# VictoriaMetrics/VictoriaLogs

Measured on NVIDIA H100. Metric: log rows scanned/sec (LogsQL phrase+regex), higher is better.
Workload: dtype u8

## Files before the change

victorialogs_b200/csrc/vl_zstd.cu:

```cuda
#include "vl_zstd.h"

#include <algorithm>
#include <array>
#include <atomic>
#include <chrono>
#include <cstdio>
#include <cstdlib>
#include <cstring>
#include <exception>
#include <thread>

#include "vl_engine.h"
#include "vl_zstd.cuh"
#include "vl_zstd_job.h"

namespace vl {

using namespace zs;

struct ZstdDev {
    DevBuf frames, blocks, bstate, huf_tab, fse_tab, huf_state, fse_state, predef, lits, seqs, frame_err, status, lists;
    bool predef_ready = false;
    cudaStream_t xstream = nullptr;
    std::vector<cudaEvent_t> events;
// ... 20 lines not shown
        hpin = nullptr; hpin_cap = 0;
    }
};

static __global__ void k_pull_words(uint4* __restrict__ dst, const uint4* __restrict__ src, size_t n) {
    for (size_t i = (size_t)blockIdx.x * blockDim.x + threadIdx.x; i < n; i += (size_t)gridDim.x * blockDim.x) dst[i] = src[i];
}
void zstd_dev_free(ZstdDev* d) { if (d) { d->release(); delete d; } }

namespace {
inline unsigned cdiv_u(uint64_t a, uint64_t b) { return (unsigned)((a + b - 1) / b); }
}

struct ZstdJob::Impl : ZstdJobImpl {};

ZstdJob::ZstdJob() : m(new Impl) {}
ZstdJob::~ZstdJob() { delete m; }
bool ZstdJob::empty() const { return m->frames.empty(); }
uint64_t ZstdJob::frames() const { return m->frames.size(); }
uint64_t ZstdJob::blocks() const { return m->blocks.size(); }
uint64_t ZstdJob::compressed_blocks() const { return m->n_compressed; }
uint64_t ZstdJob::sequences() const { return m->n_seqs; }
uint64_t ZstdJob::groups() const { return m->groups.size(); }
void ZstdJob::set_dst(uint32_t id, uint64_t arena_off) { m->frames[id].dst = arena_off; }
void ZstdJob::set_group_hook(std::function<void(uint64_t)> f) { m->group_hook = std::move(f); }

void ZstdJob::add_frame(const uint8_t* f, size_t n, uint64_t zoff, uint64_t* regen, uint32_t* id) {
    ZFrame fr{};
    zwalk::parse_frame_into(m->blocks, (uint32_t)m->frames.size(), f, n, zoff, fr);
    *regen = fr.fcs; *id = (uint32_t)m->frames.size();
    m->commit_frame(fr);
}

size_t ZstdJob::add_bytes_block(const uint8_t* p, size_t n, uint64_t zoff, uint64_t* regen, uint32_t* id) {
    ZFrame fr{};
    const size_t used = zwalk::parse_bytes_block_into(m->blocks, (uint32_t)m->frames.size(), p, n, zoff, fr);
    *regen = fr.fcs; *id = (uint32_t)m->frames.size();
    m->commit_frame(fr);
    return used;
}

void ZstdJob::add_values_blocks(const ZValuesBlock* v, size_t n, int threads, ZValuesInfo* info, size_t* bad, std::string* msg) {
    *bad = SIZE_MAX;
    if (!m->frames.empty()) throw BadInput("BUG: add_values_blocks needs an empty job");
    if (threads > 0) { m->walk_values_blocks(v, n, threads, info, bad, msg); return; }
    uint64_t total_seqs = 0;
    if (!group_scale_env()) {
        ZstdJob dry;
        dry.m->limit_scale = 1u << 20;
        for (size_t i = 0; i < n; i++) {
            try {
                uint64_t r = 0; uint32_t id = 0;
                const size_t c1 = dry.add_bytes_block(v[i].p, v[i].n, v[i].zoff, &r, &id);
                dry.add_bytes_block(v[i].p + c1, v[i].n - c1, v[i].zoff + c1, &r, &id);
            } catch (const BadInput&) { break; }
        }
        total_seqs = dry.m->n_seqs;
    }
    auto taper = [&] { if (!group_scale_env()) m->limit_scale = (m->groups.empty() || m->n_seqs > total_seqs - total_seqs / 12) ? 1 : 4; };
    for (size_t i = 0; i < n; i++) {
        try {
            uint32_t f1 = 0, f2 = 0;
            taper();
            const size_t c1 = add_bytes_block(v[i].p, v[i].n, v[i].zoff, &info[i].lens_len, &f1);
            taper();
            const size_t c2 = add_bytes_block(v[i].p + c1, v[i].n - c1, v[i].zoff + c1, &info[i].data_len, &f2);
            if (c1 + c2 != v[i].n) throw BadInput("unexpected non-empty tail after reading bytes block with strings");
        } catch (const BadInput& e) { *bad = i; *msg = e.msg; return; }
    }
    if (!group_scale_env()) m->limit_scale = 1;
}

void ZstdJob::prepare() { m->prepare(); }

void ZstdJob::digest(uint64_t out[4]) const { m->digest(out); }

void ZstdJob::run(vlscan_ctx* ctx, const uint8_t* zsrc, uint8_t* arena) {
    Impl& J = *m;
    if (J.frames.empty()) return;
    auto now = [] { return std::chrono::duration<double>(std::chrono::steady_clock::now().time_since_epoch()).count(); };
    const double t_prep = now();
    J.prepare();
    const double t_lists = now();
    const std::vector<uint32_t>& lists = J.lists;
    if (!ctx->zdev) ctx->zdev = new ZstdDev;
    ZstdDev& D = *ctx->zdev;
    cudaStream_t st = ctx->stream;
    D.frames.ensure(J.frames.size() * sizeof(ZFrame) + 16); D.blocks.ensure(J.blocks.size() * sizeof(ZBlock) + 16); D.bstate.ensure(J.blocks.size() * sizeof(ZBlockState));
    D.frame_err.ensure(J.frames.size() * 4); D.status.ensure(16); D.lists.ensure(lists.size() * 4 + 16);
    D.huf_tab.ensure(std::max<size_t>((size_t)J.max_huf * Z_HUF_TABLE * 2, 16)); D.huf_state.ensure(std::max<size_t>((size_t)J.max_huf * sizeof(ZSlotState), 16));
    D.fse_tab.ensure(std::max<size_t>((size_t)J.max_fse * Z_FSE_SLOT_BYTES, 16)); D.fse_state.ensure(std::max<size_t>((size_t)J.max_fse * sizeof(ZSlotState), 16));
    const size_t lits_stride = (J.max_lits + 64 + 255) / 256 * 256, seqs_stride = std::max<size_t>(J.max_seqs, 1);
    D.lits.ensure(2 * lits_stride); D.seqs.ensure(2 * seqs_stride * 16);
    if (!D.xstream) VL_CUDA(cudaStreamCreateWithFlags(&D.xstream, cudaStreamNonBlocking));
    if (!D.predef_ready) {
        D.predef.ensure(Z_FSE_SLOT_BYTES);
        k_zstd_predef<<<1, 32, 0, st>>>(D.predef.as<uint8_t>());
        VL_CUDA(cudaFuncSetAttribute(k_seq_decode, cudaFuncAttributeMaxDynamicSharedMemorySize, (int)(Z_SEQ_CTA_LANES * (Z_FSE_SLOT_BYTES + Z_LINEBUF))));
        VL_CUDA(cudaFuncSetAttribute(k_huf_decode, cudaFuncAttributeMaxDynamicSharedMemorySize, (int)(Z_HUF_CTA_BLOCKS * Z_HUF_TABLE * 2)));
        ctx->launches++; VL_CUDA(cudaGetLastError());
        D.predef_ready = true;
    }
    {
        auto up16 = [](size_t n) { return (n + 15) / 16 * 16; };
        const size_t nf = up16(J.frames.size() * sizeof(ZFrame)), nb = up16(J.blocks.size() * sizeof(ZBlock)), nl = up16(lists.size() * 4);
        uint8_t* h = (uint8_t*)D.ensure_hpin(nf + nb + nl + 64);
        const double t_cp = now();
        J.spread_copy(h, J.frames.data(), J.frames.size() * sizeof(ZFrame));
        J.spread_copy(h + nf, J.blocks.data(), J.blocks.size() * sizeof(ZBlock));
        if (!lists.empty()) J.spread_copy(h + nf + nb, lists.data(), lists.size() * 4);
        if (getenv("VLSCAN_DEBUG_TIMING")) fprintf(stderr, "[vlscan zstd] host: work lists of %zu launch groups %.1f ms, %.1f MB of tables to pinned memory %.1f ms (%d threads)\n",
                                                   J.groups.size(), 1e3 * (t_lists - t_prep), (nf + nb + nl) / 1e6, 1e3 * (now() - t_cp), std::max(J.threads, 1));
        k_pull_words<<<296, 256, 0, st>>>(D.frames.as<uint4>(), (const uint4*)h, nf / 16); ctx->launches++;
        k_pull_words<<<296, 256, 0, st>>>(D.blocks.as<uint4>(), (const uint4*)(h + nf), nb / 16); ctx->launches++;
        if (nl) { k_pull_words<<<296, 256, 0, st>>>(D.lists.as<uint4>(), (const uint4*)(h + nf + nb), nl / 16); ctx->launches++; }
        VL_CUDA(cudaGetLastError());
    }
    VL_CUDA(cudaMemsetAsync(D.frame_err.p, 0, J.frames.size() * 4, st));
    VL_CUDA(cudaMemsetAsync(D.status.p, 0, 16, st));
    VL_CUDA(cudaMemsetAsync(D.bstate.p, 0, J.blocks.size() * sizeof(ZBlockState), st));
    ZView V{};
    V.src = zsrc; V.arena = arena; V.frames = D.frames.as<ZFrame>(); V.blocks = D.blocks.as<ZBlock>(); V.bstate = D.bstate.as<ZBlockState>();
    V.huf_tab = D.huf_tab.as<uint16_t>(); V.fse_tab = D.fse_tab.as<uint8_t>(); V.huf_state = D.huf_state.as<ZSlotState>(); V.fse_state = D.fse_state.as<ZSlotState>();
    V.predef = D.predef.as<uint8_t>(); V.lits = D.lits.as<uint8_t>(); V.seqs = D.seqs.as<uint4>(); V.frame_err = D.frame_err.as<unsigned int>();
    V.status = D.status.as<unsigned long long>();
    const uint32_t* L = D.lists.as<uint32_t>();
    const bool dbg = getenv("VLSCAN_DEBUG_TIMING") != nullptr;
    static const char* phase_name[6] = {"huf_build", "huf_decode", "fse_build", "seq_decode", "seq_resolve", "execute"};
    std::vector<std::pair<int, std::pair<cudaEvent_t, cudaEvent_t>>> marks;
    int phase = 0;
    static const bool overlap = [] { const char* e = getenv("VLSCAN_ZSTD_OVERLAP"); return !e || atoi(e) != 0; }();
    cudaStream_t xs = overlap ? D.xstream : st;
    cudaStream_t cur_stream = st;
    auto begin = [&](int p) { phase = p; if (dbg) { cudaEvent_t a, b; cudaEventCreate(&a); cudaEventCreate(&b); cudaEventRecord(a, cur_stream); marks.push_back({p, {a, b}}); } };
    auto launched = [&] { ctx->launches++; VL_CUDA(cudaGetLastError()); if (dbg) cudaEventRecord(marks.back().second.second, cur_stream); };
    VL_CUDA(cudaEventRecord(D.event(0), st)); VL_CUDA(cudaStreamWaitEvent(xs, D.event(0), 0));
    size_t gi = 0;
    for (const Group& g : J.groups) {
        uint32_t nh = g.huf_hi - g.huf_lo, nl = g.lit_hi - g.lit_lo, ns = g.seq_hi - g.seq_lo, nf = g.frame_hi - g.frame_lo;
        if (J.group_hook) {
            uint64_t need = 0;
            for (uint32_t i = J.frames[g.frame_lo].blk_lo; i < J.frames[g.frame_hi - 1].blk_hi; i++) need = std::max<uint64_t>(need, J.blocks[i].src + (J.blocks[i].type == ZB_RLE ? 1 : J.blocks[i].size));
            J.group_hook(need);
        }
        ZView W = V;
        W.lits = V.lits + (gi & 1) * lits_stride; W.seqs = V.seqs + (gi & 1) * seqs_stride;
        cudaEvent_t ev_entropy = D.event(1 + 2 * gi), ev_exec = D.event(2 + 2 * gi);
        cur_stream = st;
        if (gi >= 2) VL_CUDA(cudaStreamWaitEvent(st, D.event(2 + 2 * (gi - 2)), 0));
        if (nh) { begin(0); k_huf_build<<<cdiv_u(nh, 4), 128, 0, st>>>(W, L + g.huf_lo, nh); launched(); }
        if (nl) { begin(1); k_huf_decode<<<cdiv_u(nl, Z_HUF_CTA_BLOCKS), Z_HUF_CTA_BLOCKS * 4, Z_HUF_CTA_BLOCKS * Z_HUF_TABLE * 2, st>>>(W, L + g.lit_lo, nl); launched(); }
        if (ns) {
            begin(2); k_fse_build<<<cdiv_u(ns, 64), 64, 0, st>>>(W, L + g.seq_lo, ns); launched();
            begin(3); k_seq_decode<<<cdiv_u(ns, Z_SEQ_CTA_LANES), 64, Z_SEQ_CTA_LANES * (Z_FSE_SLOT_BYTES + Z_LINEBUF), st>>>(W, L + g.seq_lo, ns); launched();
        }
        VL_CUDA(cudaEventRecord(ev_entropy, st));
        VL_CUDA(cudaStreamWaitEvent(xs, ev_entropy, 0));
        cur_stream = xs;
        begin(4); k_seq_resolve<<<cdiv_u(nf, 64), 64, 0, xs>>>(W, g.frame_lo, nf); launched();
        begin(5); k_execute<<<cdiv_u((uint64_t)nf * 32, Z_EXEC_WARPS * 32), Z_EXEC_WARPS * 32, 0, xs>>>(W, L + g.ord_lo, nf); launched();
        VL_CUDA(cudaEventRecord(ev_exec, xs));
        gi++;
    }
    if (gi) VL_CUDA(cudaStreamWaitEvent(st, D.event(2 + 2 * (gi - 1)), 0));
    cur_stream = st;
    if (dbg) {
        VL_CUDA(cudaStreamSynchronize(xs)); VL_CUDA(cudaStreamSynchronize(st));
        float tot[6] = {0, 0, 0, 0, 0, 0};
        for (auto& mk : marks) { float ms = 0; cudaEventElapsedTime(&ms, mk.second.first, mk.second.second); tot[mk.first] += ms; cudaEventDestroy(mk.second.first); cudaEventDestroy(mk.second.second); }
        fprintf(stderr, "[vlscan zstd] %zu groups:", J.groups.size());
        for (int p = 0; p < 6; p++) fprintf(stderr, " %s %.2f ms", phase_name[p], tot[p]);
        fprintf(stderr, "\n");
    }
    (void)phase;
    J.ran = true;
}

void ZstdJob::check(vlscan_ctx* ctx) {
    if (!m->ran) return;
    unsigned long long stt[2] = {0, 0};
    VL_CUDA(cudaMemcpyAsync(stt, ctx->zdev->status.p, 16, cudaMemcpyDeviceToHost, ctx->stream));
    VL_CUDA(cudaStreamSynchronize(ctx->stream));
    if (!stt[0]) return;
    static const char* what[] = {"", "bad Huffman tree description", "bad Huffman stream", "bad FSE table description", "bad sequences bitstream", "match offset beyond the regenerated data",
                                 "regenerated size differs from the frame content size", "bad literals section"};
    throw BadInput(std::string("cannot decompress block: ") + (stt[0] < 8 ? what[stt[0]] : "corrupted frame") + " (frame " + std::to_string(stt[1] - 1) + " of the batch)");
}

}
```

victorialogs_b200/csrc/vl_zstd.cuh:

```cuda
#pragma once
#include <cuda_runtime.h>
#include <stdint.h>
#include "vl_zstd_types.h"

namespace vl {
namespace zs {

struct ZView {
    const uint8_t* src;
    uint8_t* arena;
    const ZFrame* frames; const ZBlock* blocks; ZBlockState* bstate;
    uint16_t* huf_tab; uint8_t* fse_tab; ZSlotState* huf_state; ZSlotState* fse_state;
    const uint8_t* predef;
    uint8_t* lits; uint4* seqs;
    unsigned int* frame_err;
    unsigned long long* status;
};

static __device__ __forceinline__ void zfail(const ZView& V, uint32_t frame, unsigned code) {
    atomicCAS(&V.frame_err[frame], 0u, code);
    atomicMax(&V.status[0], (unsigned long long)code);
    atomicMax(&V.status[1], (unsigned long long)frame + 1);
}

static __device__ __forceinline__ uint64_t ldu64(const uint8_t* p) {
    uintptr_t a = (uintptr_t)p & ~(uintptr_t)7; uint32_t sh = (uint32_t)((uintptr_t)p & 7) * 8;
    uint64_t lo = *(const uint64_t*)a;
    if (!sh) return lo;
    uint64_t hi = *(const uint64_t*)(a + 8);
    return (lo >> sh) | (hi << (64 - sh));
}
static __device__ __forceinline__ uint64_t peek64(const uint8_t* base, int64_t pos) {
    if (pos >= 64) { int junk = (int)((-pos) & 7); return ldu64(base + ((pos + 7) >> 3) - 8) << junk; }
    if (pos <= 0) return 0;
    uint64_t v = 0; int nb = (int)((pos + 7) >> 3);
    for (int i = 0; i < nb; i++) v |= (uint64_t)base[i] << (8 * i);
    return v << (64 - pos);
}
struct BackReader {
    const uint8_t* base; int64_t pos; uint64_t w; int avail;
    __device__ __forceinline__ bool init(const uint8_t* p, uint32_t len) {
        base = p; w = 0; avail = 0; pos = 0;
        if (!len) return false;
        uint32_t last = p[len - 1];
        if (!last) return false;
        pos = (int64_t)len * 8 - (int64_t)(__clz(last) - 23);
        return true;
    }
    __device__ __forceinline__ uint32_t read(int n) {
        if (n == 0) return 0;
        if (n > avail) { w = peek64(base, pos); avail = 57; }
        uint32_t v = (uint32_t)(w >> (64 - n)); w <<= n; avail -= n; pos -= n;
        return v;
    }
};
struct FwdReader {
    const uint8_t* base; uint32_t len; uint32_t pos;
    __device__ __forceinline__ uint32_t read(int n) { uint32_t v = (uint32_t)(ldu64(base + (pos >> 3)) >> (pos & 7)) & ((1u << n) - 1); pos += n; return v; }
    __device__ __forceinline__ bool overrun() const { return ((pos + 7) >> 3) > len; }
};
static __device__ __forceinline__ int hibit(uint32_t v) { return 31 - __clz(v); }

static __device__ uint32_t fse_read_counts(const uint8_t* p, uint32_t len, int max_al, int max_syms, int16_t* freq, int* nsyms, int* al_out) {
    FwdReader r{p, len, 0};
    if (len < 1) return 0;
    int al = 5 + (int)r.read(4);
    if (al > max_al) return 0;
    int remaining = 1 << al, s = 0;
    while (remaining > 0 && s < max_syms) {
        if (r.overrun()) return 0;
        int bits = hibit((uint32_t)remaining + 1) + 1;
        int val = (int)r.read(bits);
        int lower = (1 << (bits - 1)) - 1;
        int thr = (1 << bits) - 1 - (remaining + 1);
        if ((val & lower) < thr) { r.pos -= 1; val &= lower; }
        else if (val > lower) val -= thr;
        int proba = val - 1;
        remaining -= proba < 0 ? -proba : proba;
        freq[s++] = (int16_t)proba;
        if (proba == 0) {
            int rep = (int)r.read(2);
            for (;;) {
                for (int i = 0; i < rep && s < max_syms; i++) freq[s++] = 0;
                if (rep != 3) break;
                if (r.overrun()) return 0;
                rep = (int)r.read(2);
            }
        }
    }
    if (remaining != 0 || r.overrun()) return 0;
    *nsyms = s; *al_out = al;
    return (r.pos + 7) >> 3;
}

static __device__ bool fse_build_table(uint32_t* tab, int al, const int16_t* freq, int nsyms, uint16_t* next) {
    const int size = 1 << al, mask = size - 1;
    int high = size;
    for (int s = 0; s < nsyms; s++) if (freq[s] == -1) { tab[--high] = (uint32_t)s; next[s] = 1; }
    const int step = (size >> 1) + (size >> 3) + 3;
    int pos = 0;
    for (int s = 0; s < nsyms; s++) {
        if (freq[s] <= 0) continue;
        next[s] = (uint16_t)freq[s];
        for (int i = 0; i < freq[s]; i++) { tab[pos] = (uint32_t)s; do { pos = (pos + step) & mask; } while (pos >= high); }
    }
    if (pos != 0) return false;
    for (int i = 0; i < size; i++) {
        uint32_t s = tab[i]; uint32_t nx = next[s]++;
        int nb = al - hibit(nx);
        uint32_t base = (nx << nb) - (uint32_t)size;
        tab[i] = s | ((uint32_t)nb << 8) | (base << 16);
    }
    return true;
}

static __device__ bool fse_build_seq_table(uint16_t* trans, uint8_t* sym, int al, const int16_t* freq, int nsyms, uint16_t* next) {
    const int size = 1 << al, mask = size - 1;
    int high = size;
    for (int s = 0; s < nsyms; s++) if (freq[s] == -1) { sym[--high] = (uint8_t)s; next[s] = 1; }
    const int step = (size >> 1) + (size >> 3) + 3;
    int pos = 0;
    for (int s = 0; s < nsyms; s++) {
        if (freq[s] <= 0) continue;
        next[s] = (uint16_t)freq[s];
        for (int i = 0; i < freq[s]; i++) { sym[pos] = (uint8_t)s; do { pos = (pos + step) & mask; } while (pos >= high); }
    }
    if (pos != 0) return false;
    for (int i = 0; i < size; i++) {
        uint32_t nx = next[sym[i]]++;
        int nb = al - hibit(nx);
        trans[i] = (uint16_t)(((nx << nb) - (uint32_t)size) | ((uint32_t)nb << 12));
    }
    return true;
}

static __device__ const int16_t Z_LL_DEFAULT[36] = {4, 3, 2, 2, 2, 2, 2, 2, 2, 2, 2, 2, 2, 1, 1, 1, 2, 2, 2, 2, 2, 2, 2, 2, 2, 3, 2, 1, 1, 1, 1, 1, -1, -1, -1, -1};
static __device__ const int16_t Z_ML_DEFAULT[53] = {1, 4, 3, 2, 2, 2, 2, 2, 2, 1, 1, 1, 1, 1, 1, 1, 1, 1, 1, 1, 1, 1, 1, 1, 1, 1, 1, 1, 1, 1, 1, 1, 1, 1, 1, 1, 1, 1, 1, 1, 1, 1, 1, 1, 1, 1, -1, -1, -1, -1, -1, -1, -1};
static __device__ const int16_t Z_OF_DEFAULT[29] = {1, 1, 1, 1, 1, 1, 2, 2, 2, 1, 1, 1, 1, 1, 1, 1, 1, 1, 1, 1, 1, 1, 1, 1, -1, -1, -1, -1, -1};
static __device__ const uint32_t Z_LL_BASE[36] = {0, 1, 2, 3, 4, 5, 6, 7, 8, 9, 10, 11, 12, 13, 14, 15, 16, 18, 20, 22, 24, 28, 32, 40, 48, 64, 128, 256, 512, 1024, 2048, 4096, 8192, 16384, 32768, 65536};
static __device__ const uint8_t Z_LL_BITS[36] = {0, 0, 0, 0, 0, 0, 0, 0, 0, 0, 0, 0, 0, 0, 0, 0, 1, 1, 1, 1, 2, 2, 3, 3, 4, 6, 7, 8, 9, 10, 11, 12, 13, 14, 15, 16};
static __device__ const uint32_t Z_ML_BASE[53] = {3, 4, 5, 6, 7, 8, 9, 10, 11, 12, 13, 14, 15, 16, 17, 18, 19, 20, 21, 22, 23, 24, 25, 26, 27, 28, 29, 30, 31, 32, 33, 34, 35, 37, 39, 41, 43, 47, 51, 59, 67, 83, 99, 131, 259, 515, 1027, 2051, 4099, 8195, 16387, 32771, 65539};
static __device__ const uint8_t Z_ML_BITS[53] = {0, 0, 0, 0, 0, 0, 0, 0, 0, 0, 0, 0, 0, 0, 0, 0, 0, 0, 0, 0, 0, 0, 0, 0, 0, 0, 0, 0, 0, 0, 0, 0, 1, 1, 1, 1, 2, 2, 3, 3, 4, 4, 5, 7, 8, 9, 10, 11, 12, 13, 14, 15, 16};

static __global__ void k_zstd_predef(uint8_t* predef) {
    if (threadIdx.x || blockIdx.x) return;
    int16_t f[53]; uint16_t nx[53];
    uint16_t* tr = (uint16_t*)predef; uint8_t* sy = predef + 2 * Z_FSE_ENTRIES;
    for (int i = 0; i < 36; i++) f[i] = Z_LL_DEFAULT[i];
    fse_build_seq_table(tr + Z_FSE_LL, sy + Z_FSE_LL, 6, f, 36, nx);
    for (int i = 0; i < 53; i++) f[i] = Z_ML_DEFAULT[i];
    fse_build_seq_table(tr + Z_FSE_ML, sy + Z_FSE_ML, 6, f, 53, nx);
    for (int i = 0; i < 29; i++) f[i] = Z_OF_DEFAULT[i];
    fse_build_seq_table(tr + Z_FSE_OF, sy + Z_FSE_OF, 5, f, 29, nx);
}

static __global__ void __launch_bounds__(128) k_huf_build(ZView V, const uint32_t* __restrict__ list, uint32_t n) {
    __shared__ uint8_t s_w[4][256];
    __shared__ uint16_t s_start[4][256];
    __shared__ int s_meta[4][4];
    const uint32_t wi = threadIdx.x >> 5, lane = threadIdx.x & 31;
    const uint32_t item = blockIdx.x * 4 + wi;
    if (item >= n) return;
    const uint32_t bi = list[item];
    const ZBlock& B = V.blocks[bi];
    const uint8_t* p = V.src + B.src + B.lit_hdr;
    const uint32_t avail = B.lit_comp;
    uint8_t* w = s_w[wi];
    if (lane == 0) {
        int ok = 1, nw = 0; uint32_t desc = 0;
        if (avail < 1) ok = 0;
        else {
            uint32_t hb = p[0];
            if (hb >= 128) {
                nw = (int)hb - 127; desc = 1 + (uint32_t)(nw + 1) / 2;
                if (desc > avail) ok = 0;
                else for (int i = 0; i < nw; i++) { uint8_t b = p[1 + i / 2]; w[i] = (i & 1) ? (b & 15) : (b >> 4); }
            } else {
                desc = 1 + hb;
                int16_t freq[256]; uint16_t nx[256]; __align__(4) uint32_t tab[64];
                int ns = 0, al = 0;
                uint32_t used = (hb == 0 || desc > avail) ? 0 : fse_read_counts(p + 1, hb, 6, 256, freq, &ns, &al);
                if (!used || used >= hb || !fse_build_table(tab, al, freq, ns, nx)) ok = 0;
                else {
                    BackReader r;
                    if (!r.init(p + 1 + used, hb - used)) ok = 0;
                    else {
                        uint32_t s1 = r.read(al), s2 = r.read(al);
                        for (;;) {
                            if (nw >= 254) { ok = 0; break; }
                            uint32_t e1 = tab[s1]; w[nw++] = (uint8_t)e1; s1 = (e1 >> 16) + r.read((e1 >> 8) & 0xFF);
                            if (r.pos < 0) { w[nw++] = (uint8_t)tab[s2]; break; }
                            if (nw >= 254) { ok = 0; break; }
                            uint32_t e2 = tab[s2]; w[nw++] = (uint8_t)e2; s2 = (e2 >> 16) + r.read((e2 >> 8) & 0xFF);
                            if (r.pos < 0) { w[nw++] = (uint8_t)tab[s1]; break; }
                        }
                    }
                }
            }
        }
        int maxbits = 0;
        if (ok) {
            uint32_t sum = 0;
            for (int i = 0; i < nw; i++) { if (w[i] > 11) { ok = 0; break; } if (w[i]) sum += 1u << (w[i] - 1); }
            if (ok && sum == 0) ok = 0;
            if (ok) {
                maxbits = hibit(sum) + 1;
                uint32_t left = (1u << maxbits) - sum;
                if (maxbits > 11 || (left & (left - 1)) != 0) ok = 0;
                else { w[nw++] = (uint8_t)(hibit(left) + 1); }
            }
        }
        if (ok) {
            uint32_t cnt[13]; for (int i = 0; i < 13; i++) cnt[i] = 0;
            for (int i = 0; i < nw; i++) cnt[w[i]]++;
            uint32_t nxt[13]; uint32_t acc = 0;
            for (int k = 1; k <= maxbits; k++) { nxt[k] = acc; acc += cnt[k] << (k - 1); }
            for (int i = 0; i < nw; i++) if (w[i]) { s_start[wi][i] = (uint16_t)nxt[w[i]]; nxt[w[i]] += 1u << (w[i] - 1); }
        }
        s_meta[wi][0] = nw; s_meta[wi][1] = maxbits; s_meta[wi][2] = ok;
        V.bstate[bi].huf_desc_len = desc;
    }
    __syncwarp();
    if (!s_meta[wi][2]) { if (lane == 0) zfail(V, B.frame, ZERR_HUF_DESC); return; }
    const int nw = s_meta[wi][0], maxbits = s_meta[wi][1];
    uint16_t* tab = V.huf_tab + (size_t)B.huf_own * Z_HUF_TABLE;
    for (int s = (int)lane; s < nw; s += 32) {
        uint32_t ww = w[s];
        if (!ww) continue;
        uint32_t len = 1u << (ww - 1), st = s_start[wi][s];
        uint16_t e = (uint16_t)(s | ((maxbits + 1 - ww) << 8));
        for (uint32_t k = 0; k < len; k++) tab[st + k] = e;
    }
    if (lane == 0) V.huf_state[B.huf_own].huf_maxbits = (uint8_t)maxbits;
}

static const uint32_t Z_HUF_CTA_BLOCKS = 56;
static __global__ void __launch_bounds__(Z_HUF_CTA_BLOCKS * 4) k_huf_decode(ZView V, const uint32_t* __restrict__ list, uint32_t n) {
    extern __shared__ uint16_t s_tab[];
    const uint32_t local = threadIdx.x >> 2, k = threadIdx.x & 3;
    const uint32_t first = blockIdx.x * Z_HUF_CTA_BLOCKS;
    const uint32_t here = min(Z_HUF_CTA_BLOCKS, n - first);
    for (uint32_t it = 0; it < here; it++) {
        const ZBlock& Bt = V.blocks[list[first + it]];
        const uint32_t entries = 1u << V.huf_state[Bt.huf_slot].huf_maxbits;
        const uint4* g = (const uint4*)(V.huf_tab + (size_t)Bt.huf_slot * Z_HUF_TABLE);
        uint4* d = (uint4*)(s_tab + (size_t)it * Z_HUF_TABLE);
        for (uint32_t e = threadIdx.x; e < entries / 8; e += blockDim.x) d[e] = g[e];
        if (entries < 8 && threadIdx.x == 0) d[0] = g[0];
    }
    __syncthreads();
    if (local >= here) return;
    const uint32_t bi = list[first + local];
    const ZBlock& B = V.blocks[bi];
    if (V.frame_err[B.frame]) return;
    if (B.lit_streams == 1 && k) return;
    const uint32_t maxbits = V.huf_state[B.huf_slot].huf_maxbits;
    const uint16_t* tab = s_tab + (size_t)local * Z_HUF_TABLE;
    const uint32_t desc = B.lit_type == ZL_COMPRESSED ? V.bstate[bi].huf_desc_len : 0;
    if (maxbits == 0 || desc > B.lit_comp) { zfail(V, B.frame, ZERR_HUF_STREAM); return; }
    const uint8_t* s = V.src + B.src + B.lit_hdr + desc;
    uint32_t total = B.lit_comp - desc, len, nout;
    uint8_t* out = V.lits + B.lit_off;
    if (B.lit_streams == 1) { len = total; nout = B.lit_regen; }
    else {
        if (total < 6) { if (!k) zfail(V, B.frame, ZERR_HUF_STREAM); return; }
        uint32_t s1 = s[0] | (s[1] << 8), s2 = s[2] | (s[3] << 8), s3 = s[4] | (s[5] << 8);
        if ((uint64_t)6 + s1 + s2 + s3 > total) { if (!k) zfail(V, B.frame, ZERR_HUF_STREAM); return; }
        uint32_t seg = (B.lit_regen + 3) / 4;
        if (3 * seg > B.lit_regen) { if (!k) zfail(V, B.frame, ZERR_HUF_STREAM); return; }
        uint32_t off = 6 + (k > 0 ? s1 : 0) + (k > 1 ? s2 : 0) + (k > 2 ? s3 : 0);
        len = k == 0 ? s1 : k == 1 ? s2 : k == 2 ? s3 : total - 6 - s1 - s2 - s3;
        s += off; out += (size_t)k * seg; nout = k < 3 ? seg : B.lit_regen - 3 * seg;
    }
    if (!len || !s[len - 1]) { zfail(V, B.frame, ZERR_HUF_STREAM); return; }
    int64_t pos = (int64_t)len * 8 - (int64_t)(__clz((uint32_t)s[len - 1]) - 23);
    const int sh = 64 - (int)maxbits;
    uint32_t i = 0;
    while (i < nout && (((uintptr_t)(out + i)) & 7) && pos >= 0) { const uint32_t e = tab[peek64(s, pos) >> sh]; pos -= (int64_t)(e >> 8); out[i++] = (uint8_t)e; }
    if (nout - i >= 8 && pos >= 128) {
        const uint64_t* org = (const uint64_t*)((uintptr_t)s & ~(uintptr_t)7);
        const uint32_t s0 = (uint32_t)((uintptr_t)s & 7) * 8;
        uint32_t ab = s0 + (uint32_t)pos;
        uint32_t k = (ab - 1) >> 6;
        uint64_t hi = org[k], lo = org[(int32_t)k - 1], n1 = org[(int32_t)k - 2], n2 = org[(int32_t)k - 3];
        const uint32_t sh32 = 32 - maxbits;
        while (nout - i >= 8 && ab - s0 >= 128) {
            uint64_t acc = 0;
#pragma unroll
            for (int half = 0; half < 2; half++) {
                const uint32_t sft = (0u - ab) & 63u;
                const bool up = sft < 32;
                const uint32_t a = up ? (uint32_t)(hi >> 32) : (uint32_t)hi, b = up ? (uint32_t)hi : (uint32_t)(lo >> 32), c = up ? (uint32_t)(lo >> 32) : (uint32_t)lo;
                uint32_t ch = __funnelshift_l(b, a, sft), cl = __funnelshift_l(c, b, sft);
                uint32_t used = 0;
#pragma unroll
                for (int q = 0; q < 4; q++) {
                    const uint32_t e = tab[ch >> sh32];
                    const uint32_t nb = e >> 8;
                    ch = __funnelshift_l(cl, ch, nb); cl <<= nb;
                    used += nb;
                    acc |= (uint64_t)(e & 0xFF) << (8 * (4 * half + q));
                }
                ab -= used;
                const uint32_t k2 = (ab - 1) >> 6;
                if (k2 != k) { hi = lo; lo = n1; n1 = n2; n2 = org[(int32_t)k2 - 3]; k = k2; }
            }
            *(uint64_t*)(out + i) = acc; i += 8;
        }
        pos = (int64_t)ab - (int64_t)s0;
    }
    while (i < nout && pos >= 0) { const uint32_t e = tab[peek64(s, pos) >> sh]; pos -= (int64_t)(e >> 8); out[i++] = (uint8_t)e; }
    if (i != nout || pos != 0) zfail(V, B.frame, ZERR_HUF_STREAM);
}

static __global__ void __launch_bounds__(64) k_fse_build(ZView V, const uint32_t* __restrict__ list, uint32_t n) {
    const uint32_t t = blockIdx.x * blockDim.x + threadIdx.x;
    if (t >= n) return;
    const uint32_t bi = list[t];
    const ZBlock& B = V.blocks[bi];
    const uint8_t* p = V.src + B.src;
    uint32_t off = B.seq_hdr + 1;
    bool ok = off <= B.size && (B.modes & 3) == 0;
    int16_t freq[53]; uint16_t nx[53];
    ZSlotState st{0, 0, 0, 0};
    for (int k = 0; k < 3 && ok; k++) {
        int mode = k == 0 ? (B.modes >> 6) & 3 : k == 1 ? (B.modes >> 4) & 3 : (B.modes >> 2) & 3;
        int max_al = k == 1 ? 8 : 9, max_syms = k == 0 ? 36 : k == 1 ? 32 : 53;
        uint32_t toff = k == 0 ? Z_FSE_LL : k == 1 ? Z_FSE_OF : Z_FSE_ML;
        int al = 0;
        if (mode == 1) {
            if (off + 1 > B.size) { ok = false; break; }
            uint32_t sym = p[off++];
            if ((int)sym >= max_syms) { ok = false; break; }
            uint8_t* slot = V.fse_tab + (size_t)B.fse_own * Z_FSE_SLOT_BYTES;
            ((uint16_t*)slot)[toff] = 0; slot[2 * Z_FSE_ENTRIES + toff] = (uint8_t)sym;
        } else if (mode == 2) {
            int ns = 0;
            uint32_t used = off < B.size ? fse_read_counts(p + off, B.size - off, max_al, max_syms, freq, &ns, &al) : 0;
            uint8_t* slot = V.fse_tab + (size_t)B.fse_own * Z_FSE_SLOT_BYTES;
            if (!used || !fse_build_seq_table((uint16_t*)slot + toff, slot + 2 * Z_FSE_ENTRIES + toff, al, freq, ns, nx)) { ok = false; break; }
            off += used;
        } else continue;
        if (k == 0) st.ll_al = (uint8_t)al; else if (k == 1) st.of_al = (uint8_t)al; else st.ml_al = (uint8_t)al;
    }
    if (!ok || off > B.size) { zfail(V, B.frame, ZERR_FSE_DESC); return; }
    if (B.fse_own != Z_PREDEF) V.fse_state[B.fse_own] = st;
    V.bstate[bi].seq_bits_off = off;
}

static const uint32_t Z_SEQ_CTA_LANES = 56;
static const uint32_t Z_LINEBUF = 272;
static const uint32_t Z_SEQ_LEAD = 160;
static __device__ __forceinline__ uint32_t lds_u32(uint32_t sa) { uint32_t v; asm volatile("ld.shared.u32 %0, [%1];" : "=r"(v) : "r"(sa)); return v; }
static __device__ __forceinline__ uint32_t bfe_u32(uint32_t a, uint32_t pos, uint32_t len) { uint32_t d; asm("bfe.u32 %0, %1, %2, %3;" : "=r"(d) : "r"(a), "r"(pos), "r"(len)); return d; }
static __device__ __forceinline__ uint32_t top_bits(uint32_t x, uint32_t n) { return __funnelshift_rc(x, 0u, 32u - n); }
struct SeqLane {
    const uint8_t* gorg;
    uint32_t ring;
    uint32_t p;
    uint32_t fc;
    const uint16_t* tr; const uint8_t* sy; const uint32_t* llv; const uint32_t* mlv;
    uint32_t sl, so, sm, r1, r2, r3, ndirty, sum_ll, sum_ml, sticky;
    uint4* out;
    __device__ __forceinline__ void fetch_chunk() {
        fc--;
        const uint32_t sa = ring + ((fc & 15u) << 4);
        const uint8_t* g = gorg + (size_t)fc * 16;
        asm volatile("cp.async.cg.shared.global [%0], [%1], 16;" ::"r"(sa), "l"(g) : "memory");
    }
    __device__ __forceinline__ void window(uint32_t& c2, uint32_t& c1, uint32_t& c0) const {
        const uint32_t k = (p - 1u) >> 5, s = (0u - p) & 31u;
        const uint32_t w3 = lds_u32(ring + ((k << 2) & 252u)), w2 = lds_u32(ring + (((k - 1u) << 2) & 252u));
        const uint32_t w1 = lds_u32(ring + (((k - 2u) << 2) & 252u)), w0 = lds_u32(ring + (((k - 3u) << 2) & 252u));
        c2 = __funnelshift_l(w2, w3, s); c1 = __funnelshift_l(w1, w2, s); c0 = __funnelshift_l(w0, w1, s);
    }
    template <bool LAST>
    __device__ __forceinline__ void step() {
        const uint32_t tl = tr[sl], to = tr[so], tm = tr[sm];
        const uint32_t oc = sy[so], vl = llv[sy[sl]], vm = mlv[sy[sm]];
        if (p < fc * 128u + Z_SEQ_LEAD * 8u && fc > 0) fetch_chunk();
        asm volatile("cp.async.commit_group;\n\tcp.async.wait_group 3;" ::: "memory");
        uint32_t c2, c1, c0;
        window(c2, c1, c0);
        const uint32_t nL = vl >> 24, nM = vm >> 24, n2 = nM + nL;
        const uint32_t ov = (1u << oc) + top_bits(c2, oc);
        const uint32_t v2 = top_bits(__funnelshift_l(c1, c2, oc), n2);
        const uint32_t ml = (vm & 0xFFFFFFu) + (v2 >> nL), ll = (vl & 0xFFFFFFu) + bfe_u32(v2, 0, nL);
        const uint32_t o3 = oc + n2;
        if (!LAST) {
            const uint32_t bL = tl >> 12, bM = tm >> 12, bO = to >> 12, n3 = bL + bM + bO;
            const bool up = o3 < 32;
            const uint32_t v3 = top_bits(__funnelshift_l(up ? c1 : c0, up ? c2 : c1, o3), n3);
            sl = Z_FSE_LL + (tl & 0xFFFu) + (v3 >> (bM + bO));
            sm = Z_FSE_ML + (tm & 0xFFFu) + bfe_u32(v3, bO, bM);
            so = Z_FSE_OF + (to & 0xFFFu) + bfe_u32(v3, 0, bO);
            p -= o3 + n3;
        } else p -= o3;
        uint32_t o;
        if (ov > 3) { o = ov - 3; r3 = r2; r2 = r1; r1 = o; }
        else {
            const uint32_t idx = ov + (ll == 0 ? 1 : 0);
            if (idx == 1) o = r1;
            else {
                o = idx == 2 ? r2 : idx == 3 ? r3 : (r1 == 0xFFFFFFFFu ? r1 : r1 - 1);
                if (idx != 2) r3 = r2;
                r2 = r1; r1 = o;
            }
        }
        ndirty += (r1 | r2 | r3) >> 31;
        *out++ = make_uint4(ll, ml, o, ov);
        sum_ll += ll; sum_ml += ml;
        sticky |= p | sum_ll | sum_ml;
    }
};
static __global__ void __launch_bounds__(64) k_seq_decode(ZView V, const uint32_t* __restrict__ list, uint32_t n) {
    extern __shared__ __align__(16) uint8_t s_fse[];
    __shared__ uint32_t s_llv[36], s_mlv[53];
    const uint32_t first = blockIdx.x * Z_SEQ_CTA_LANES;
    const uint32_t here = min(Z_SEQ_CTA_LANES, n - first);
    if (threadIdx.x < 36) s_llv[threadIdx.x] = Z_LL_BASE[threadIdx.x] | ((uint32_t)Z_LL_BITS[threadIdx.x] << 24);
    if (threadIdx.x < 53) s_mlv[threadIdx.x] = Z_ML_BASE[threadIdx.x] | ((uint32_t)Z_ML_BITS[threadIdx.x] << 24);
    for (uint32_t it = 0; it < here; it++) {
        const ZBlock& Bt = V.blocks[list[first + it]];
        const uint4* src_ll = (const uint4*)(Bt.ll_slot == Z_PREDEF ? V.predef : V.fse_tab + (size_t)Bt.ll_slot * Z_FSE_SLOT_BYTES);
        const uint4* src_ml = (const uint4*)(Bt.ml_slot == Z_PREDEF ? V.predef : V.fse_tab + (size_t)Bt.ml_slot * Z_FSE_SLOT_BYTES);
        const uint4* src_of = (const uint4*)(Bt.of_slot == Z_PREDEF ? V.predef : V.fse_tab + (size_t)Bt.of_slot * Z_FSE_SLOT_BYTES);
        uint4* d = (uint4*)(s_fse + (size_t)it * Z_FSE_SLOT_BYTES);
        for (uint32_t c = threadIdx.x; c < Z_FSE_SLOT_BYTES / 16; c += blockDim.x) {
            const uint4* src = c < 64 ? src_ll : c < 128 ? src_ml : c < 160 ? src_of : c < 192 ? src_ll : c < 224 ? src_ml : src_of;
            d[c] = src[c];
        }
    }
    __syncthreads();
    if (threadIdx.x >= here) return;
    const uint32_t bi = list[first + threadIdx.x];
    const ZBlock& B = V.blocks[bi];
    if (V.frame_err[B.frame]) return;
    const uint32_t off = V.bstate[bi].seq_bits_off;
    const int ll_al = B.ll_slot == Z_PREDEF ? 6 : V.fse_state[B.ll_slot].ll_al;
    const int of_al = B.of_slot == Z_PREDEF ? 5 : V.fse_state[B.of_slot].of_al;
    const int ml_al = B.ml_slot == Z_PREDEF ? 6 : V.fse_state[B.ml_slot].ml_al;
    if (off >= B.size) { zfail(V, B.frame, ZERR_SEQ_STREAM); return; }
    const uint64_t st = B.src + off;
    const uint32_t len = B.size - off;
    const uint32_t last = V.src[st + len - 1];
    if (!last) { zfail(V, B.frame, ZERR_SEQ_STREAM); return; }
    SeqLane L;
    const uint64_t org = (st & ~255ull) - 256;
    const uint32_t s0 = (uint32_t)(st - org) * 8;
    L.gorg = V.src + org;
    L.ring = (uint32_t)__cvta_generic_to_shared(s_fse + (size_t)Z_SEQ_CTA_LANES * Z_FSE_SLOT_BYTES + (size_t)threadIdx.x * Z_LINEBUF);
    L.p = s0 + len * 8 - (uint32_t)(__clz(last) - 23);
    L.fc = ((L.p - 1u) >> 7) + 1u;
#pragma unroll
    for (int q = 0; q < 12; q++) L.fetch_chunk();
    asm volatile("cp.async.commit_group;\n\tcp.async.wait_group 0;" ::: "memory");
    L.tr = (const uint16_t*)(s_fse + (size_t)threadIdx.x * Z_FSE_SLOT_BYTES);
    L.sy = s_fse + (size_t)threadIdx.x * Z_FSE_SLOT_BYTES + 2 * Z_FSE_ENTRIES;
    L.llv = s_llv; L.mlv = s_mlv;
    {
        uint32_t c2, c1, c0;
        L.window(c2, c1, c0);
        L.sl = Z_FSE_LL + top_bits(c2, ll_al);
        L.so = Z_FSE_OF + top_bits(__funnelshift_l(c1, c2, ll_al), of_al);
        L.sm = Z_FSE_ML + top_bits(__funnelshift_l(c1, c2, ll_al + of_al), ml_al);
        L.p -= ll_al + of_al + ml_al;
        (void)c0;
    }
    const uint32_t DIRTY = 0xFFFFFFFFu;
    L.r1 = B.rep_known ? 1 : DIRTY; L.r2 = B.rep_known ? 4 : DIRTY; L.r3 = B.rep_known ? 8 : DIRTY;
    L.ndirty = 0; L.sum_ll = 0; L.sum_ml = 0; L.sticky = L.p;
    L.out = V.seqs + B.seq_base;
    const uint32_t nseq = B.nseq;
    for (uint32_t i = 0; i + 1 < nseq; i++) L.step<false>();
    if (nseq) L.step<true>();
    asm volatile("cp.async.wait_group 0;" ::: "memory");
    if ((L.sticky >> 31) || L.p != s0 || L.sum_ll > B.lit_regen) { zfail(V, B.frame, ZERR_SEQ_STREAM); return; }
    ZBlockState& S = V.bstate[bi];
    S.out_len = B.lit_regen + L.sum_ml;
    S.clean_from = B.rep_known ? 0 : L.ndirty + 1;
    S.rep[0] = L.r1; S.rep[1] = L.r2; S.rep[2] = L.r3;
}

static __global__ void __launch_bounds__(64) k_seq_resolve(ZView V, uint32_t frame_lo, uint32_t nframes) {
    const uint32_t t = blockIdx.x * blockDim.x + threadIdx.x;
    if (t >= nframes) return;
    const uint32_t f = frame_lo + t;
    if (V.frame_err[f]) return;
    const ZFrame& F = V.frames[f];
    uint64_t out = 0;
    uint32_t r1 = 1, r2 = 4, r3 = 8;
    for (uint32_t bi = F.blk_lo; bi < F.blk_hi; bi++) {
        const ZBlock& B = V.blocks[bi];
        ZBlockState& S = V.bstate[bi];
        S.out_base = (uint32_t)out;
        if (B.type != ZB_COMPRESSED) { out += B.size; S.out_len = B.size; continue; }
        if (!B.nseq) { S.out_len = B.lit_regen; out += B.lit_regen; }
        else {
            uint4* __restrict__ sq = V.seqs + B.seq_base;
            const uint32_t redo = min(S.clean_from, B.nseq);
            for (uint32_t i = 0; i < redo; i++) {
                uint4 q = sq[i];
                uint32_t ll = q.x, ov = q.w, o;
                if (ov > 3) { o = ov - 3; r3 = r2; r2 = r1; r1 = o; }
                else {
                    uint32_t idx = ov + (ll == 0 ? 1 : 0);
                    if (idx == 1) o = r1;
                    else {
                        o = idx == 2 ? r2 : idx == 3 ? r3 : r1 - 1;
                        if (idx != 2) r3 = r2;
                        r2 = r1; r1 = o;
                    }
                }
                sq[i].z = o;
            }
            if (S.clean_from <= B.nseq) { r1 = S.rep[0]; r2 = S.rep[1]; r3 = S.rep[2]; }
            out += S.out_len;
        }
        if (out > F.fcs) { zfail(V, f, ZERR_SIZE); return; }
    }
    if (out != F.fcs) zfail(V, f, ZERR_SIZE);
}

static const uint32_t Z_RING = 4096;
static const uint32_t Z_EXEC_WARPS = 4;
static __device__ __forceinline__ uint32_t ldu32(const uint8_t* p) {
    const uintptr_t a = (uintptr_t)p & ~(uintptr_t)3;
    const uint32_t lo = *(const uint32_t*)a, hi = *(const uint32_t*)(a + 4);
    return __funnelshift_r(lo, hi, (uint32_t)((uintptr_t)p & 3) * 8);
}
static __global__ void __launch_bounds__(128) k_execute(ZView V, const uint32_t* __restrict__ order, uint32_t nframes) {
    __shared__ __align__(16) uint8_t s_ring[Z_EXEC_WARPS][Z_RING];
    const uint32_t wid = (blockIdx.x * blockDim.x + threadIdx.x) >> 5, lane = threadIdx.x & 31;
    if (wid >= nframes) return;
    const uint32_t f = order[wid];
    if (V.frame_err[f]) return;
    const ZFrame& F = V.frames[f];
    uint8_t* dst = V.arena + F.dst;
    uint8_t* ring = s_ring[threadIdx.x >> 5];
    const uint32_t abase = (uint32_t)(uintptr_t)dst;
#define VL_RIDX(p) ((abase + (p)) & (Z_RING - 1))
#define VL_RING(p) ring[VL_RIDX(p)]
    uint32_t ring_lo = 0;
    for (uint32_t bi = F.blk_lo; bi < F.blk_hi; bi++) {
        const ZBlock& B = V.blocks[bi];
        const uint32_t blk_base = V.bstate[bi].out_base;
        const uint8_t* p = V.src + B.src;
        if (B.type == ZB_RAW) { for (uint32_t k = lane; k < B.size; k += 32) { uint8_t v = p[k]; dst[blk_base + k] = v; VL_RING(blk_base + k) = v; } __syncwarp(); continue; }
        if (B.type == ZB_RLE) { uint8_t v = p[0]; for (uint32_t k = lane; k < B.size; k += 32) { dst[blk_base + k] = v; VL_RING(blk_base + k) = v; } __syncwarp(); continue; }
        const uint8_t* lit = B.lit_type == ZL_RAW ? p + B.lit_hdr : V.lits + B.lit_off;
        const bool lit_rle = B.lit_type == ZL_RLE;
        const uint8_t rle_byte = lit_rle ? p[B.lit_hdr] : 0;
        const uint4* __restrict__ sq = V.seqs + B.seq_base;
        uint32_t lit_run = 0, out_run = blk_base;
        uint4 qn = lane < B.nseq ? sq[lane] : make_uint4(0, 0, 0, 0);
        for (uint32_t g = 0; g < B.nseq; g += 32) {
            const uint4 q = qn;
            qn = g + 32 + lane < B.nseq ? sq[g + 32 + lane] : make_uint4(0, 0, 0, 0);
            uint32_t il = q.x, io = q.x + q.y;
#pragma unroll
            for (int d = 1; d < 32; d <<= 1) { uint32_t a = __shfl_up_sync(0xffffffffu, il, d), b = __shfl_up_sync(0xffffffffu, io, d); if ((int)lane >= d) { il += a; io += b; } }
            const uint32_t lit_start = il - q.x;
            const uint32_t o_start = io - q.x - q.y;
            const uint32_t T = __shfl_sync(0xffffffffu, il, 31), O = __shfl_sync(0xffffffffu, io, 31);
            const uint32_t gend = out_run + O;
            const uint32_t cnt = min(32u, B.nseq - g);
            const uint32_t ml = q.y, off = q.z, amd = out_run + o_start + q.x;
            if (__any_sync(0xffffffffu, lane < cnt && (off == 0 || off > amd))) { if (lane == 0) zfail(V, f, ZERR_OFFSET); return; }
            const uint32_t s_src = amd - off, e_src = s_src + min(ml, off);
            int dep = -1;
            {
                uint32_t lo = 0;
#pragma unroll
                for (int s = 16; s; s >>= 1) { uint32_t v = __shfl_sync(0xffffffffu, amd, (lo + s - 1) & 31); if ((lo + s - 1) < cnt && v < e_src) lo += s; }
                const uint32_t ci = (lo - 1) & 31;
                const uint32_t ca = __shfl_sync(0xffffffffu, amd, ci), cm = __shfl_sync(0xffffffffu, ml, ci);
                if (lo > 0 && ca + cm > s_src) dep = (int)lo - 1;
            }
            if (O < Z_RING) {
                uint32_t cl = (q.x + 3) >> 2, cm = (ml + 3) >> 2;
#pragma unroll
                for (int d = 1; d < 32; d <<= 1) { uint32_t a = __shfl_up_sync(0xffffffffu, cl, d), b = __shfl_up_sync(0xffffffffu, cm, d); if ((int)lane >= d) { cl += a; cm += b; } }
                const uint32_t CL = __shfl_sync(0xffffffffu, cl, 31);
                const uint32_t pk = lit_start | (o_start << 16);
                const uint8_t* lsrc = lit + lit_run;
                for (uint32_t c0 = 0; c0 < CL; c0 += 128) {
                    uint32_t w[4], at[4], nb[4];
#pragma unroll
                    for (int u = 0; u < 4; u++) {
                        nb[u] = 0; w[u] = 0; at[u] = 0;
                        if (c0 + 32 * u >= CL) continue;
                        const uint32_t c = c0 + 32 * u + lane;
                        uint32_t lo = 0;
#pragma unroll
                        for (int s = 16; s; s >>= 1) { uint32_t x = __shfl_sync(0xffffffffu, cl, (lo + s - 1) & 31); if (x <= c) lo += s; }
                        const uint32_t jc = __shfl_sync(0xffffffffu, cl, lo & 31), jl = __shfl_sync(0xffffffffu, q.x, lo & 31), jp = __shfl_sync(0xffffffffu, pk, lo & 31);
                        if (c < CL) {
                            const uint32_t b0 = (c - (jc - ((jl + 3) >> 2))) * 4;
                            nb[u] = min(4u, jl - b0);
                            w[u] = lit_rle ? rle_byte * 0x01010101u : ldu32(lsrc + (jp & 0xFFFF) + b0);
                            at[u] = out_run + (jp >> 16) + b0;
                        }
                    }
#pragma unroll
                    for (int u = 0; u < 4; u++) {
#pragma unroll
                        for (int t = 0; t < 4; t++) if ((uint32_t)t < nb[u]) VL_RING(at[u] + t) = (uint8_t)(w[u] >> (8 * t));
                    }
                }
                __syncwarp();
                uint32_t cur = 0;
                while (cur < cnt) {
// ... 103 lines not shown
```

victorialogs_b200/csrc/vl_zstd_types.h:

```cpp
#pragma once
#include <stdint.h>

namespace vl {
namespace zs {

enum { ZERR_NONE = 0, ZERR_HUF_DESC = 1, ZERR_HUF_STREAM = 2, ZERR_FSE_DESC = 3, ZERR_SEQ_STREAM = 4, ZERR_OFFSET = 5, ZERR_SIZE = 6, ZERR_LITERALS = 7 };
enum { ZB_RAW = 0, ZB_RLE = 1, ZB_COMPRESSED = 2 };
enum { ZL_RAW = 0, ZL_RLE = 1, ZL_COMPRESSED = 2, ZL_TREELESS = 3 };
static const uint32_t Z_PREDEF = 0xFFFFFFFFu;
static const uint32_t Z_HUF_TABLE = 2048;
static const uint32_t Z_FSE_LL = 0, Z_FSE_ML = 512, Z_FSE_OF = 1024, Z_FSE_ENTRIES = 1280, Z_FSE_SLOT_BYTES = 3 * 1280;

struct ZFrame {
    uint64_t dst;
    uint64_t fcs;
    uint32_t blk_lo, blk_hi;
};
struct ZBlock {
    uint64_t src;
    uint64_t lit_off;
    uint64_t seq_base;
    uint32_t size;
    uint32_t frame;
    uint32_t lit_hdr;
    uint32_t lit_regen, lit_comp;
    uint32_t nseq;
    uint32_t seq_hdr;
    uint32_t huf_slot;
    uint32_t huf_own;
    uint32_t fse_own;
    uint32_t ll_slot, of_slot, ml_slot;
    uint8_t type, lit_type, lit_streams, modes;
    uint8_t rep_known;
    uint8_t pad[3];
};
struct ZBlockState {
    uint32_t huf_desc_len;
    uint32_t seq_bits_off;
    uint32_t out_len;
    uint32_t out_base;
    uint32_t clean_from;
    uint32_t rep[3];
};
struct ZSlotState { uint8_t huf_maxbits, ll_al, of_al, ml_al; };

}
}
```

Measured before the change: 21.70 billion.

## Pack FSE sequence tables into 16-bit entries and stage them with cp.async

The FSE sequence decode table now stores symbol and next-state counter in one 16-bit entry, and the bit count and base are derived at decode time with clz. The separate symbol byte array goes away and per-slot shared memory shrinks from 3840 to 2560 bytes. With the smaller slots the kernel raises lanes per CTA from 56 to 80 and threads from 64 to 96. Table staging is reworked so each block's slot pointers are gathered in parallel and the copies use cp.async instead of a serial per-block loop. The decode step does a few more ALU operations per sequence in exchange for fewer shared loads and a smaller footprint.

After: 21.70 billion, median of 6. Within noise of the previous version (-0.0%).

```diff
diff --git a/victorialogs_b200/csrc/vl_zstd.cu b/victorialogs_b200/csrc/vl_zstd.cu
--- a/victorialogs_b200/csrc/vl_zstd.cu
+++ b/victorialogs_b200/csrc/vl_zstd.cu
@@ -196,7 +196,7 @@
         if (nl) { begin(1); k_huf_decode<<<cdiv_u(nl, Z_HUF_CTA_BLOCKS), Z_HUF_CTA_BLOCKS * 4, Z_HUF_CTA_BLOCKS * Z_HUF_TABLE * 2, st>>>(W, L + g.lit_lo, nl); launched(); }
         if (ns) {
             begin(2); k_fse_build<<<cdiv_u(ns, 64), 64, 0, st>>>(W, L + g.seq_lo, ns); launched();
-            begin(3); k_seq_decode<<<cdiv_u(ns, Z_SEQ_CTA_LANES), 64, Z_SEQ_CTA_LANES * (Z_FSE_SLOT_BYTES + Z_LINEBUF), st>>>(W, L + g.seq_lo, ns); launched();
+            begin(3); k_seq_decode<<<cdiv_u(ns, Z_SEQ_CTA_LANES), Z_SEQ_CTA_THREADS, Z_SEQ_CTA_LANES * (Z_FSE_SLOT_BYTES + Z_LINEBUF), st>>>(W, L + g.seq_lo, ns); launched();
         }
         VL_CUDA(cudaEventRecord(ev_entropy, st));
         VL_CUDA(cudaStreamWaitEvent(xs, ev_entropy, 0));
diff --git a/victorialogs_b200/csrc/vl_zstd.cuh b/victorialogs_b200/csrc/vl_zstd.cuh
--- a/victorialogs_b200/csrc/vl_zstd.cuh
+++ b/victorialogs_b200/csrc/vl_zstd.cuh
@@ -114,22 +114,21 @@
     return true;
 }
 
-static __device__ bool fse_build_seq_table(uint16_t* trans, uint8_t* sym, int al, const int16_t* freq, int nsyms, uint16_t* next) {
+static __device__ bool fse_build_seq_table(uint16_t* tab, int al, const int16_t* freq, int nsyms, uint16_t* next) {
     const int size = 1 << al, mask = size - 1;
     int high = size;
-    for (int s = 0; s < nsyms; s++) if (freq[s] == -1) { sym[--high] = (uint8_t)s; next[s] = 1; }
+    for (int s = 0; s < nsyms; s++) if (freq[s] == -1) { tab[--high] = (uint16_t)s; next[s] = 1; }
     const int step = (size >> 1) + (size >> 3) + 3;
     int pos = 0;
     for (int s = 0; s < nsyms; s++) {
         if (freq[s] <= 0) continue;
         next[s] = (uint16_t)freq[s];
-        for (int i = 0; i < freq[s]; i++) { sym[pos] = (uint8_t)s; do { pos = (pos + step) & mask; } while (pos >= high); }
+        for (int i = 0; i < freq[s]; i++) { tab[pos] = (uint16_t)s; do { pos = (pos + step) & mask; } while (pos >= high); }
     }
     if (pos != 0) return false;
     for (int i = 0; i < size; i++) {
-        uint32_t nx = next[sym[i]]++;
-        int nb = al - hibit(nx);
-        trans[i] = (uint16_t)(((nx << nb) - (uint32_t)size) | ((uint32_t)nb << 12));
+        const uint32_t s = tab[i];
+        tab[i] = (uint16_t)(next[s]++ | (s << 10));
     }
     return true;
 }
@@ -145,13 +144,13 @@
 static __global__ void k_zstd_predef(uint8_t* predef) {
     if (threadIdx.x || blockIdx.x) return;
     int16_t f[53]; uint16_t nx[53];
-    uint16_t* tr = (uint16_t*)predef; uint8_t* sy = predef + 2 * Z_FSE_ENTRIES;
+    uint16_t* tab = (uint16_t*)predef;
     for (int i = 0; i < 36; i++) f[i] = Z_LL_DEFAULT[i];
-    fse_build_seq_table(tr + Z_FSE_LL, sy + Z_FSE_LL, 6, f, 36, nx);
+    fse_build_seq_table(tab + Z_FSE_LL, 6, f, 36, nx);
     for (int i = 0; i < 53; i++) f[i] = Z_ML_DEFAULT[i];
-    fse_build_seq_table(tr + Z_FSE_ML, sy + Z_FSE_ML, 6, f, 53, nx);
+    fse_build_seq_table(tab + Z_FSE_ML, 6, f, 53, nx);
     for (int i = 0; i < 29; i++) f[i] = Z_OF_DEFAULT[i];
-    fse_build_seq_table(tr + Z_FSE_OF, sy + Z_FSE_OF, 5, f, 29, nx);
+    fse_build_seq_table(tab + Z_FSE_OF, 5, f, 29, nx);
 }
 
 static __global__ void __launch_bounds__(128) k_huf_build(ZView V, const uint32_t* __restrict__ list, uint32_t n) {
@@ -332,13 +331,13 @@
             if (off + 1 > B.size) { ok = false; break; }
             uint32_t sym = p[off++];
             if ((int)sym >= max_syms) { ok = false; break; }
-            uint8_t* slot = V.fse_tab + (size_t)B.fse_own * Z_FSE_SLOT_BYTES;
-            ((uint16_t*)slot)[toff] = 0; slot[2 * Z_FSE_ENTRIES + toff] = (uint8_t)sym;
+            uint16_t* slot = (uint16_t*)(V.fse_tab + (size_t)B.fse_own * Z_FSE_SLOT_BYTES);
+            slot[toff] = (uint16_t)(1u | (sym << 10));
         } else if (mode == 2) {
             int ns = 0;
             uint32_t used = off < B.size ? fse_read_counts(p + off, B.size - off, max_al, max_syms, freq, &ns, &al) : 0;
-            uint8_t* slot = V.fse_tab + (size_t)B.fse_own * Z_FSE_SLOT_BYTES;
-            if (!used || !fse_build_seq_table((uint16_t*)slot + toff, slot + 2 * Z_FSE_ENTRIES + toff, al, freq, ns, nx)) { ok = false; break; }
+            uint16_t* slot = (uint16_t*)(V.fse_tab + (size_t)B.fse_own * Z_FSE_SLOT_BYTES);
+            if (!used || !fse_build_seq_table(slot + toff, al, freq, ns, nx)) { ok = false; break; }
             off += used;
         } else continue;
         if (k == 0) st.ll_al = (uint8_t)al; else if (k == 1) st.of_al = (uint8_t)al; else st.ml_al = (uint8_t)al;
@@ -348,7 +347,8 @@
     V.bstate[bi].seq_bits_off = off;
 }
 
-static const uint32_t Z_SEQ_CTA_LANES = 56;
+static const uint32_t Z_SEQ_CTA_LANES = 80;
+static const uint32_t Z_SEQ_CTA_THREADS = 96;
 static const uint32_t Z_LINEBUF = 272;
 static const uint32_t Z_SEQ_LEAD = 160;
 static __device__ __forceinline__ uint32_t lds_u32(uint32_t sa) { uint32_t v; asm volatile("ld.shared.u32 %0, [%1];" : "=r"(v) : "r"(sa)); return v; }
@@ -359,7 +359,8 @@
     uint32_t ring;
     uint32_t p;
     uint32_t fc;
-    const uint16_t* tr; const uint8_t* sy; const uint32_t* llv; const uint32_t* mlv;
+    const uint16_t* tab; const uint32_t* llv; const uint32_t* mlv;
+    uint32_t aL, aM, aO, kL, kM, kO;
     uint32_t sl, so, sm, r1, r2, r3, ndirty, sum_ll, sum_ml, sticky;
     uint4* out;
     __device__ __forceinline__ void fetch_chunk() {
@@ -376,8 +377,8 @@
     }
     template <bool LAST>
     __device__ __forceinline__ void step() {
-        const uint32_t tl = tr[sl], to = tr[so], tm = tr[sm];
-        const uint32_t oc = sy[so], vl = llv[sy[sl]], vm = mlv[sy[sm]];
+        const uint32_t el = tab[sl], eo = tab[so], em = tab[sm];
+        const uint32_t oc = eo >> 10, vl = llv[el >> 10], vm = mlv[em >> 10];
         if (p < fc * 128u + Z_SEQ_LEAD * 8u && fc > 0) fetch_chunk();
         asm volatile("cp.async.commit_group;\n\tcp.async.wait_group 3;" ::: "memory");
         uint32_t c2, c1, c0;
@@ -388,12 +389,13 @@
         const uint32_t ml = (vm & 0xFFFFFFu) + (v2 >> nL), ll = (vl & 0xFFFFFFu) + bfe_u32(v2, 0, nL);
         const uint32_t o3 = oc + n2;
         if (!LAST) {
-            const uint32_t bL = tl >> 12, bM = tm >> 12, bO = to >> 12, n3 = bL + bM + bO;
+            const uint32_t xL = el & 0x3FFu, xM = em & 0x3FFu, xO = eo & 0x3FFu;
+            const uint32_t bL = (uint32_t)__clz(xL) + aL, bM = (uint32_t)__clz(xM) + aM, bO = (uint32_t)__clz(xO) + aO, n3 = bL + bM + bO;
             const bool up = o3 < 32;
             const uint32_t v3 = top_bits(__funnelshift_l(up ? c1 : c0, up ? c2 : c1, o3), n3);
-            sl = Z_FSE_LL + (tl & 0xFFFu) + (v3 >> (bM + bO));
-            sm = Z_FSE_ML + (tm & 0xFFFu) + bfe_u32(v3, bO, bM);
-            so = Z_FSE_OF + (to & 0xFFFu) + bfe_u32(v3, 0, bO);
+            sl = (xL << bL) + kL + (v3 >> (bM + bO));
+            sm = (xM << bM) + kM + bfe_u32(v3, bO, bM);
+            so = (xO << bO) + kO + bfe_u32(v3, 0, bO);
             p -= o3 + n3;
         } else p -= o3;
         uint32_t o;
@@ -413,24 +415,28 @@
         sticky |= p | sum_ll | sum_ml;
     }
 };
-static __global__ void __launch_bounds__(64) k_seq_decode(ZView V, const uint32_t* __restrict__ list, uint32_t n) {
+static __global__ void __launch_bounds__(Z_SEQ_CTA_THREADS) k_seq_decode(ZView V, const uint32_t* __restrict__ list, uint32_t n) {
     extern __shared__ __align__(16) uint8_t s_fse[];
     __shared__ uint32_t s_llv[36], s_mlv[53];
     const uint32_t first = blockIdx.x * Z_SEQ_CTA_LANES;
     const uint32_t here = min(Z_SEQ_CTA_LANES, n - first);
     if (threadIdx.x < 36) s_llv[threadIdx.x] = Z_LL_BASE[threadIdx.x] | ((uint32_t)Z_LL_BITS[threadIdx.x] << 24);
     if (threadIdx.x < 53) s_mlv[threadIdx.x] = Z_ML_BASE[threadIdx.x] | ((uint32_t)Z_ML_BITS[threadIdx.x] << 24);
-    for (uint32_t it = 0; it < here; it++) {
-        const ZBlock& Bt = V.blocks[list[first + it]];
-        const uint4* src_ll = (const uint4*)(Bt.ll_slot == Z_PREDEF ? V.predef : V.fse_tab + (size_t)Bt.ll_slot * Z_FSE_SLOT_BYTES);
-        const uint4* src_ml = (const uint4*)(Bt.ml_slot == Z_PREDEF ? V.predef : V.fse_tab + (size_t)Bt.ml_slot * Z_FSE_SLOT_BYTES);
-        const uint4* src_of = (const uint4*)(Bt.of_slot == Z_PREDEF ? V.predef : V.fse_tab + (size_t)Bt.of_slot * Z_FSE_SLOT_BYTES);
-        uint4* d = (uint4*)(s_fse + (size_t)it * Z_FSE_SLOT_BYTES);
-        for (uint32_t c = threadIdx.x; c < Z_FSE_SLOT_BYTES / 16; c += blockDim.x) {
-            const uint4* src = c < 64 ? src_ll : c < 128 ? src_ml : c < 160 ? src_of : c < 192 ? src_ll : c < 224 ? src_ml : src_of;
-            d[c] = src[c];
-        }
-    }
+    __shared__ const uint8_t* s_slot[3][Z_SEQ_CTA_LANES];
+    if (threadIdx.x < here) {
+        const ZBlock& Bt = V.blocks[list[first + threadIdx.x]];
+        s_slot[0][threadIdx.x] = Bt.ll_slot == Z_PREDEF ? V.predef : V.fse_tab + (size_t)Bt.ll_slot * Z_FSE_SLOT_BYTES;
+        s_slot[1][threadIdx.x] = Bt.ml_slot == Z_PREDEF ? V.predef : V.fse_tab + (size_t)Bt.ml_slot * Z_FSE_SLOT_BYTES;
+        s_slot[2][threadIdx.x] = Bt.of_slot == Z_PREDEF ? V.predef : V.fse_tab + (size_t)Bt.of_slot * Z_FSE_SLOT_BYTES;
+    }
+    __syncthreads();
+    const uint32_t s_base = (uint32_t)__cvta_generic_to_shared(s_fse);
+    for (uint32_t u = threadIdx.x; u < here * (Z_FSE_SLOT_BYTES / 16); u += blockDim.x) {
+        const uint32_t it = u / (Z_FSE_SLOT_BYTES / 16), c = u - it * (Z_FSE_SLOT_BYTES / 16);
+        const uint8_t* g = s_slot[c < 64 ? 0 : c < 128 ? 1 : 2][it] + (size_t)c * 16;
+        asm volatile("cp.async.cg.shared.global [%0], [%1], 16;" ::"r"(s_base + u * 16), "l"(g) : "memory");
+    }
+    asm volatile("cp.async.commit_group;\n\tcp.async.wait_group 0;" ::: "memory");
     __syncthreads();
     if (threadIdx.x >= here) return;
     const uint32_t bi = list[first + threadIdx.x];
@@ -455,9 +461,10 @@
 #pragma unroll
     for (int q = 0; q < 12; q++) L.fetch_chunk();
     asm volatile("cp.async.commit_group;\n\tcp.async.wait_group 0;" ::: "memory");
-    L.tr = (const uint16_t*)(s_fse + (size_t)threadIdx.x * Z_FSE_SLOT_BYTES);
-    L.sy = s_fse + (size_t)threadIdx.x * Z_FSE_SLOT_BYTES + 2 * Z_FSE_ENTRIES;
+    L.tab = (const uint16_t*)(s_fse + (size_t)threadIdx.x * Z_FSE_SLOT_BYTES);
     L.llv = s_llv; L.mlv = s_mlv;
+    L.aL = (uint32_t)(ll_al - 31); L.aM = (uint32_t)(ml_al - 31); L.aO = (uint32_t)(of_al - 31);
+    L.kL = Z_FSE_LL - (1u << ll_al); L.kM = Z_FSE_ML - (1u << ml_al); L.kO = Z_FSE_OF - (1u << of_al);
     {
         uint32_t c2, c1, c0;
         L.window(c2, c1, c0);
diff --git a/victorialogs_b200/csrc/vl_zstd_types.h b/victorialogs_b200/csrc/vl_zstd_types.h
--- a/victorialogs_b200/csrc/vl_zstd_types.h
+++ b/victorialogs_b200/csrc/vl_zstd_types.h
@@ -9,7 +9,7 @@
 enum { ZL_RAW = 0, ZL_RLE = 1, ZL_COMPRESSED = 2, ZL_TREELESS = 3 };
 static const uint32_t Z_PREDEF = 0xFFFFFFFFu;
 static const uint32_t Z_HUF_TABLE = 2048;
-static const uint32_t Z_FSE_LL = 0, Z_FSE_ML = 512, Z_FSE_OF = 1024, Z_FSE_ENTRIES = 1280, Z_FSE_SLOT_BYTES = 3 * 1280;
+static const uint32_t Z_FSE_LL = 0, Z_FSE_ML = 512, Z_FSE_OF = 1024, Z_FSE_ENTRIES = 1280, Z_FSE_SLOT_BYTES = 2 * 1280;
 
 struct ZFrame {
     uint64_t dst;
```
